# harveybc/gym-fx

Hardware: AMD Instinct MI355X
Metric: env-steps/sec (whole node) PPO EURUSD-1m 4096 vec-envs (higher is better)
Workload: dtype bf16; 1 GPU; model=PPO MLP(256,256) actor-critic bf16 MFMA, global_batch=524288, seq_len=32, parallelism=dp1, n_envs_per_gpu=4096, rollout_steps=128, obs_dim=260, preprocessor=feature_window_preprocessor, reward=pnl_reward, pairs=1

## Files before the change

### gymfx_amd/algo/ppo.py

```python
from __future__ import annotations

import time
from dataclasses import dataclass
from typing import Any, Dict, List

import torch

from ..envs.vec_env import VecFxEnv
from ..models.lstm import ActorCriticLSTM
from ..models.mlp import ActorCriticMLP
from ..ops import api


@dataclass
class PPOConfig:
    rollout_steps: int = 128
    ppo_epochs: int = 4
    minibatches: int = 8
    gamma: float = 0.99
    gae_lambda: float = 0.95
    clip_eps: float = 0.2
    ent_coef: float = 0.01
    vf_coef: float = 0.5
    lr: float = 3e-4
    max_grad_norm: float = 0.5
    seed: int = 0
    hidden: int = 256
    normalize_adv: bool = True
    shuffle_rows: bool = True
    use_graphs: bool = True
    policy: str = "mlp"
    bptt_len: int = 16
    fused_rollout: bool = False
    rollout_streams: int = 1
    fuse_sample: bool = True
    fuse_head: bool = False
    overlap_gather: bool = False
    fused_opt_tail: bool = True
    fused_head_bwd: bool = True

    @classmethod
    def from_config(cls, cfg: Dict[str, Any]) -> "PPOConfig":
        out = cls()
        mapping = {
            "rollout_steps": "rollout_steps",
            "ppo_epochs": "ppo_epochs",
            "minibatches": "minibatches",
            "gamma": "gamma",
            "gae_lambda": "gae_lambda",
            "clip_eps": "clip_eps",
            "ent_coef": "ent_coef",
            "vf_coef": "vf_coef",
            "lr": "learning_rate",
            "max_grad_norm": "max_grad_norm",
            "hidden": "hidden_size",
            "normalize_adv": "normalize_adv",
            "shuffle_rows": "shuffle_rows",
            "use_graphs": "use_graphs",
            "policy": "policy_model",
            "bptt_len": "bptt_len",
            "rollout_streams": "rollout_streams",
            "fused_rollout": "fused_rollout",
            "fuse_sample": "fuse_sample",
            "fuse_head": "fuse_head",
            "overlap_gather": "overlap_gather",
            "fused_opt_tail": "fused_opt_tail",
            "fused_head_bwd": "fused_head_bwd",
        }
        from ..config.merger import convert_type

        for attr, key in mapping.items():
            if cfg.get(key) is not None:
                cur = getattr(out, attr)
                val = convert_type(cfg[key]) if isinstance(cur, bool) else cfg[key]
                setattr(out, attr, type(cur)(val))
        if cfg.get("seed") is not None:
            out.seed = int(cfg["seed"])
        return out


class PPOTrainer:
    def __init__(self, env: VecFxEnv, cfg: PPOConfig, *, rank: int = 0,
                 world_size: int = 1, process_group=None):
        self.env = env
        self.cfg = cfg
        self.rank = rank
        self.world_size = world_size
        self.pg = process_group
        self.device = env.device
        if getattr(env.params, "action_space_mode", "discrete") != "discrete":
            raise ValueError(
                "PPO training uses the 3-way discrete head; set "
                "action_space_mode='discrete' (continuous mode is for "
                "external agents driving the env, reference "
                "env.py:343-360 coercion semantics)")

        N = env.n_envs
        T = cfg.rollout_steps
        D = env.obs_dim
        self.N, self.T, self.D = N, T, D
# ... 79 lines not shown
            self.logp_mb_s = [torch.empty(M, dtype=torch.float32, device=dev)
                              for _ in range(ns)]
            self.adv_mb_s = [torch.empty(M, dtype=torch.float32, device=dev)
                             for _ in range(ns)]
            self.ret_mb_s = [torch.empty(M, dtype=torch.float32, device=dev)
                             for _ in range(ns)]
            self.obs_mb = self.obs_mb_s[0]
            self.act_mb = self.act_mb_s[0]
            self.logp_mb = self.logp_mb_s[0]
            self.adv_mb = self.adv_mb_s[0]
            self.ret_mb = self.ret_mb_s[0]

        self.step_base = torch.zeros((), dtype=torch.int64, device=dev)
        self.mb_ctr = torch.zeros((), dtype=torch.int64, device=dev)
        self.sample_seed = cfg.seed * 1_000_003 + rank
        self.shuffle_seed = cfg.seed * 9973 + rank

        import os as _os
        self._fuse_gather = (
            not self.recurrent and self.device.type == "cuda"
            and cfg.shuffle_rows and not self._overlap
            and _os.environ.get("GYMFX_FUSE_GATHER", "0") == "1")
        self._fm = {"seed": self.shuffle_seed, "minibatches": cfg.minibatches,
                    "ctr_off": -1, "step_base": self.step_base,
                    "mb_ctr": self.mb_ctr}

        self._fused_tail = bool(cfg.fused_opt_tail) and (
            not self.recurrent
            or _os.environ.get("GYMFX_LSTM_OPT_TAIL", "0") == "1")
        self.model.fused_tail = self._fused_tail
        self.model.fuse_norm = (self._fused_tail and world_size <= 1
                                and cfg.max_grad_norm > 0)
        self._fused_head = bool(cfg.fused_head_bwd) and not self.recurrent
        self._loss_shards = (
            torch.zeros(64, 32, dtype=torch.float32, device=dev)
            if self._fused_head and self.device.type == "cuda" else None)
        self._mb_ticket = (
            torch.zeros((), dtype=torch.int32, device=dev)
            if self._fused_tail
            and _os.environ.get("GYMFX_GATHER_TICKET", "0") == "1" else None)

        self.global_step = 0
        self.update_count = 0
        self.use_graphs = bool(cfg.use_graphs) and self.device.type == "cuda"
        self._split = (self.device.type == "cuda" and cfg.rollout_streams > 1
                       and N % 2 == 0)
        self._fused = (self.device.type == "cuda" and cfg.fused_rollout
                       and not self.recurrent and cfg.hidden == 256)
        self._fuse_sample = (self.device.type == "cuda" and cfg.fuse_sample
                             and getattr(env, "_native", None) is not None
                             and env.params.action_space_mode != "continuous")
        self._fuse_head = (self._fuse_sample and cfg.fuse_head
                           and cfg.hidden % 8 == 0 and n_actions + 1 <= 8
                           and not cfg.fused_rollout)
        if self._split:
            self._s2 = torch.cuda.Stream()
            self.acts_half = [self.model.alloc_acts(N // 2),
                              self.model.alloc_acts(N // 2)]
        if self._overlap:
            self._gs = torch.cuda.Stream()
        self._graphs_ready = False
        self.g_rollout = None
        self.g_gather = None
        self.g_fwd_bwd = None
        self.g_opt = None
        from ..parallel.ddp import GradAllReducer
# ... 466 lines not shown
```

### gymfx_amd/config/defaults.py

```python
from __future__ import annotations

DEFAULT_VALUES = {
    "mode": "inference",
    "driver_mode": "buy_hold",
    "steps": 500,

    "data_feed_plugin": "default_data_feed",
    "broker_plugin": "default_broker",
    "strategy_plugin": "default_strategy",
    "preprocessor_plugin": "default_preprocessor",
    "reward_plugin": "pnl_reward",
    "metrics_plugin": "default_metrics",

    "input_data_file": "examples/data/eurusd.csv",
    "date_column": "DATE_TIME",
    "price_column": "CLOSE",
    "instrument": "EUR_USD",
    "timeframe": "M1",
    "headers": True,
    "max_rows": None,

    "window_size": 32,
    "initial_cash": 10000.0,
    "position_size": 1.0,
# ... 18 lines not shown
    "n_envs": 1,
    "device": "auto",
    "seed": None,
    "autoreset": False,
    "env_start_mode": "zero",
    "action_space_mode": "discrete",
    "continuous_action_threshold": 0.33,
    "min_equity": None,
    "financing_enabled": False,
    "rollover_rate_data": None,
    "financing_rate_data_file": None,
    "rollover_hour_utc": 22,
    "enforce_margin_preflight": False,

    "policy_model": "mlp",
    "hidden_size": 256,
    "rollout_steps": 128,
    "ppo_epochs": 4,
    "minibatches": 8,
    "bptt_len": 16,
    "learning_rate": 3e-4,
    "gamma": 0.99,
    "gae_lambda": 0.95,
    "clip_eps": 0.2,
    "ent_coef": 0.01,
    "vf_coef": 0.5,
    "max_grad_norm": 0.5,
    "train_updates": 10,
    "use_graphs": True,
    "fuse_sample": True,
    "overlap_gather": False,
    "fused_opt_tail": True,
    "fused_head_bwd": True,
    "checkpoint_file": None,
    "checkpoint_interval": 0,
    "resume": False,
    "trace_file": None,

    "serve_host": "127.0.0.1",
    "serve_port": 8400,

    "optimization_trials": 16,
    "optimization_steps": 256,
    "optimization_refine_trials": 0,
}
```

### gymfx_amd/models/mlp.py

```python
from __future__ import annotations

import math
from dataclasses import dataclass
from typing import Dict, Optional, Tuple

import torch

from ..ops import api


@dataclass
class _ParamSlice:
    name: str
    shape: Tuple[int, ...]
    sl: slice
    is_weight: bool


class ActorCriticMLP:
    def __init__(
        self,
        obs_dim: int,
        n_actions: int = 3,
        hidden: int = 256,
# ... 24 lines not shown
        self.n_params = off

        g = torch.Generator().manual_seed(seed)
        flat = torch.empty(off, dtype=torch.float32)
        for name, shape, is_w in dims:
            s = self.slices[name]
            if is_w:
                fan_in = shape[0]
                bound = 1.0 / math.sqrt(fan_in)
                flat[s.sl] = (torch.rand(s.sl.stop - s.sl.start, generator=g) * 2 - 1) * bound
            else:
                flat[s.sl] = 0.0
        self.params = flat.to(device)
        self.grads = torch.zeros_like(self.params)
        self.m = torch.zeros_like(self.params)
        self.v = torch.zeros_like(self.params)
        self.params_bf16 = self.params.to(torch.bfloat16)
        self._wt: Dict[str, torch.Tensor] = {}
        for name in ("W1", "W2", "W3"):
            s = self.slices[name]
            K_, N_ = s.shape
            self._wt[name] = torch.empty(N_, K_, dtype=torch.bfloat16, device=device)
        self._refresh_wt()
        self.adam_step = 0
        self.adam_ctr = torch.zeros((), dtype=torch.int32, device=device)
        self._clip_part = torch.zeros(256, dtype=torch.float32, device=device)
        self._clip_scale = torch.ones(1, dtype=torch.float32, device=device)
        self._wg_ws: Dict[str, Tuple[torch.Tensor, Optional[torch.Tensor]]] = {}
        self.wgrad_slabs = 64
        self.fused_tail = False
        self.fuse_norm = False
        self._adam_ticket = torch.zeros((), dtype=torch.int32, device=device)
        self._fin_segs = None

    def w(self, name: str) -> torch.Tensor:
        s = self.slices[name]
        return self.params_bf16[s.sl].view(*s.shape)

    def wt(self, name: str) -> torch.Tensor:
        return self._wt[name]

    def _refresh_wt(self) -> None:
        for name, t in self._wt.items():
            api.transpose_bf16(self.w(name), t)

    def f32(self, name: str) -> torch.Tensor:
        s = self.slices[name]
        return self.params[s.sl].view(*s.shape)

    def grad(self, name: str) -> torch.Tensor:
        s = self.slices[name]
        return self.grads[s.sl].view(*s.shape)

    def _wg_slabs(self, K: int, N: int) -> int:
        import os
        ov = os.environ.get("GYMFX_WGRAD_SLABS")
        if ov:
            return int(ov)
        tiles = ((K + 63) // 64) * ((N + 63) // 64)
        s = self.wgrad_slabs
        while tiles * s < 2048:
            s *= 2
        return s

    def _finalize_segments(self):
        if self._fin_segs is None:
# ... 5 lines not shown
                segs.append((db, N, S, self.slices[bn].sl.start, True))
            self._fin_segs = segs
        return self._fin_segs

    def _wg_workspace(self, name: str, K: int, N: int, want_db: bool):
        key = f"{name}:{K}x{N}"
        if key not in self._wg_ws:
            S = self._wg_slabs(K, N)
            dw = torch.empty(S, K, N, dtype=torch.float32, device=self.device)
            db = torch.empty(S, N, dtype=torch.float32, device=self.device) if want_db else None
            self._wg_ws[key] = (dw, db, S)
        return self._wg_ws[key]

    def alloc_acts(self, M: int) -> Dict[str, torch.Tensor]:
        dev = self.device
        return {
            "h1": torch.empty(M, self.hidden, dtype=torch.bfloat16, device=dev),
            "h2": torch.empty(M, self.hidden, dtype=torch.bfloat16, device=dev),
            "head": torch.empty(M, self.head_dim, dtype=torch.float32, device=dev),
        }

    def fused_step(self, obs_bf16: torch.Tensor, actions: torch.Tensor,
                   logp: torch.Tensor, value: torch.Tensor, *, seed: int,
                   step: int, step_base: torch.Tensor, row_offset: int = 0,
                   greedy: bool = False) -> None:
        from ..ops import native
        native.require().mlp_policy_rollout(
            obs_bf16, self.wt("W1"), self.f32("b1"), self.wt("W2"),
            self.f32("b2"), self.wt("W3"), self.f32("b3"), actions, logp,
            value, seed, step, step_base, row_offset, greedy)

    def forward(self, obs_bf16: torch.Tensor, acts: Dict[str, torch.Tensor],
                a_feistel: "Optional[dict]" = None) -> torch.Tensor:
        api.gemm(obs_bf16, self.wt("W1"), self.f32("b1"), acts["h1"], act=2,
                 trans_b=True, a_perm=a_feistel)
        api.gemm(acts["h1"], self.wt("W2"), self.f32("b2"), acts["h2"], act=2, trans_b=True)
        api.gemm(acts["h2"], self.wt("W3"), self.f32("b3"), acts["head"], act=0, trans_b=True)
        return acts["head"]

    def forward_hidden(self, obs_bf16: torch.Tensor,
                       acts: Dict[str, torch.Tensor]) -> torch.Tensor:
        api.gemm(obs_bf16, self.wt("W1"), self.f32("b1"), acts["h1"], act=2, trans_b=True)
        api.gemm(acts["h1"], self.wt("W2"), self.f32("b2"), acts["h2"], act=2, trans_b=True)
        return acts["h2"]

    def head_loss_backward(
        self,
        acts: Dict[str, torch.Tensor],
        actions: torch.Tensor,
        old_logp: torch.Tensor,
        adv: torch.Tensor,
        ret: torch.Tensor,
        dhead: torch.Tensor,
        scratch: Dict[str, torch.Tensor],
        *,
        clip_eps: float,
        ent_coef: float,
        vf_coef: float,
        inv_count: float,
        losses: Optional[torch.Tensor] = None,
    ) -> None:
        dw_p, db_p, slabs = self._wg_workspace("W3", self.hidden, self.head_dim, True)
        api.head_loss_bwd(
            acts["h2"], self.wt("W3"), self.w("W3"), self.f32("b3"), actions,
            old_logp, adv, ret, acts["head"], dhead, scratch["dh2"],
            self.grad("W3"), self.grad("b3"), workspace=(dw_p, db_p),
            slabs=slabs, reduce=not self.fused_tail, clip_eps=clip_eps,
            ent_coef=ent_coef, vf_coef=vf_coef, inv_count=inv_count,
            losses=losses)

    def backward(
        self,
        obs_bf16: torch.Tensor,
        acts: Dict[str, torch.Tensor],
        dhead: torch.Tensor,
        scratch: Dict[str, torch.Tensor],
        a_feistel: "Optional[dict]" = None,
        skip_head: bool = False,
    ) -> None:
        M = dhead.shape[0]
        dh2 = scratch["dh2"]
        dh1 = scratch["dh1"]
        red = not self.fused_tail
        if not skip_head:
            dw_p, db_p, slabs = self._wg_workspace("W3", self.hidden, self.head_dim, True)
            api.wgrad(acts["h2"], dhead, self.grad("W3"), self.grad("b3"),
                      workspace=(dw_p, db_p), slabs=slabs, reduce=red)
            api.gemm(dhead, self.w("W3"), None, dh2, Yact=acts["h2"], trans_b=True,
                     act=1, dact_tanh=True)
        dw_p, db_p, slabs = self._wg_workspace("W2", self.hidden, self.hidden, True)
        api.wgrad(acts["h1"], dh2, self.grad("W2"), self.grad("b2"),
                  workspace=(dw_p, db_p), slabs=slabs, reduce=red)
        api.gemm(dh2, self.w("W2"), None, dh1, Yact=acts["h1"], trans_b=True,
                 act=1, dact_tanh=True)
        dw_p, db_p, slabs = self._wg_workspace("W1", self.obs_dim, self.hidden, True)
        api.wgrad(obs_bf16, dh1, self.grad("W1"), self.grad("b1"),
                  workspace=(dw_p, db_p), slabs=slabs, x_perm=a_feistel,
                  reduce=red)
        if self.fused_tail:
            api.grads_finalize(self._finalize_segments(), self.grads,
                               self._clip_part if self.fuse_norm else None)

    def alloc_scratch(self, M: int) -> Dict[str, torch.Tensor]:
        dev = self.device
        return {
            "dh2": torch.empty(M, self.hidden, dtype=torch.bfloat16, device=dev),
            "dh1": torch.empty(M, self.hidden, dtype=torch.bfloat16, device=dev),
        }

    def adam(self, lr: float, *, beta1=0.9, beta2=0.999, eps=1e-8,
             max_grad_norm: float = 0.0) -> None:
        self.adam_step += 1
        clip = None
        if max_grad_norm and max_grad_norm > 0:
            clip = (self._clip_part, max_grad_norm)
        if self.fused_tail:
            api.adam_tail(self.params, self.grads, self.m, self.v,
                          self.params_bf16, lr=lr, beta1=beta1, beta2=beta2,
                          eps=eps, step_ctr=self.adam_ctr,
                          ticket=self._adam_ticket, clip=clip,
                          sumsq_done=self.fuse_norm,
                          mirrors=[(self.slices[n].sl.start, t)
                                   for n, t in self._wt.items()])
            return
        api.adam(self.params, self.grads, self.m, self.v, self.params_bf16,
                 lr=lr, beta1=beta1, beta2=beta2, eps=eps, step=self.adam_step,
                 step_ctr=self.adam_ctr, clip=clip)
# ... 26 lines not shown
```

### gymfx_amd/ops/api.py

```python
from __future__ import annotations

from typing import Optional, Sequence, Tuple

import os

import torch

from . import native

_LSTM_FUSED = os.environ.get("GYMFX_LSTM_FUSED", "1") != "0"
_LSTM_BWD_FUSED = os.environ.get("GYMFX_LSTM_BWD_FUSED", "0") == "1"


def _use_native(t: torch.Tensor) -> bool:
    if t.is_cuda:
        native.require()
        return True
    return False



def gemm(
    A: torch.Tensor,
    B: torch.Tensor,
    bias: Optional[torch.Tensor],
    C: torch.Tensor,
    *,
    Yact: Optional[torch.Tensor] = None,
    trans_b: bool = False,
    act: int = 1,
    dact_tanh: bool = False,
    accum: bool = False,
    a_perm: "Optional[dict]" = None,
) -> torch.Tensor:
    if _use_native(A):
        if a_perm is not None:
            native.require().gemm(A, B, bias, C, Yact, trans_b, act,
                                  dact_tanh, accum,
                                  ap_seed=a_perm["seed"],
                                  ap_minibatches=a_perm["minibatches"],
                                  ap_ctr_off=a_perm.get("ctr_off", 0),
                                  ap_step_base=a_perm["step_base"],
                                  ap_mb_ctr=a_perm["mb_ctr"])
            return C
        native.require().gemm(A, B, bias, C, Yact, trans_b, act, dact_tanh,
                              accum)
        return C
    if a_perm is not None:
        A = A[_perm_rows(A.shape[0], C.shape[0], a_perm)]
    a = A.to(torch.float32)
    b = B.to(torch.float32)
    if trans_b:
        b = b.t()
    out = a @ b
    if bias is not None:
        out = out + bias
    if act == 2:
        out = torch.tanh(out)
    if dact_tanh:
        y = Yact.to(torch.float32)
        out = out * (1.0 - y * y)
    if act == 0:
        if accum:
            C.add_(out)
        else:
            C.copy_(out)
    else:
        C.copy_(out.to(torch.bfloat16))
# ... 662 lines not shown
```

### gymfx_amd/ops/csrc/bindings.cpp

```cpp
#include <torch/extension.h>

#include <c10/hip/HIPStream.h>
#include <hip/hip_runtime.h>

#include <unordered_map>
#include <string>
#include <vector>

#include "env_common.h"
#include "mfma_dispatch.h"

namespace gymfx {

void launch_env_step(const EnvPtrs& P, const EnvParamsK& K, int env_lo,
                     int env_cnt, hipStream_t stream);
void launch_build_obs(const EnvPtrs& P, const EnvParamsK& K, int env_lo,
                      int env_cnt, hipStream_t stream);
void launch_env_step_obs(const EnvPtrs& P, const EnvParamsK& K, int env_lo,
                         int env_cnt, hipStream_t stream);
void launch_gemm(const void* A, const void* B, const float* bias, void* C,
                 const void* Yact, int M, int N, int K, bool trans_b, int act,
                 bool dact_tanh, bool add_bias, bool accum, hipStream_t stream,
                 const FeistelMap* fmp = nullptr);
void launch_lstm_cell_fwd(const void* gates_pre, const void* gates_h,
                          const float* c_prev, float* c_new, void* h_new,
                          const bool* done, void* h_masked, float* c_masked,
                          void* acts_out, int64_t M, int H,
                          hipStream_t stream);
void launch_lstm_cell_bwd(const void* acts, const float* c_prev,
                          const float* c_new, const void* dh_head,
                          const float* dh_next, const float* dc_next,
                          const bool* done, void* dgates, float* dc_prev,
                          int64_t M, int H, hipStream_t stream);
bool launch_lstm_gemm_cell_fwd(const void* A, const void* B,
                               const void* gates_pre, void* acts_out,
                               const float* c_prev, float* c_new, void* h_new,
                               const bool* done, void* h_masked,
                               float* c_masked, int M, int N, int K,
                               hipStream_t stream);
bool launch_lstm_bwd_fused(const void* acts, const float* c_prev,
                           const float* c_new, const void* dh_head,
                           const float* dh_next, const float* dc_next,
                           const bool* done, const void* B, void* dgates,
                           float* dc_prev, float* dh_prev, int M, int H,
                           hipStream_t stream);
void launch_mask_reset(void* h, float* c, const bool* done, int64_t M, int H,
                       hipStream_t stream);
void launch_masked_state(const void* h_raw, const float* c_raw,
                         const bool* done, void* h_in, float* c_in, int64_t M,
                         int H, hipStream_t stream);
void launch_mb_gather_seq(const void* obs_src, const int64_t* act_src,
                          const float* logp_src, const float* adv_src,
                          const float* ret_src, const bool* done_src,
                          const float* h0_src,
                          const float* c0_src, void* obs_mb, int64_t* act_mb,
                          float* logp_mb, float* adv_mb, float* ret_mb,
// ... 494 lines not shown
  const int N = trans_b ? (int)B.size(0) : (int)B.size(1);
  TORCH_CHECK((trans_b ? B.size(1) : B.size(0)) == K, "gemm K mismatch");
  TORCH_CHECK(C.size(1) == N && (C.size(0) == M || ap_step_base.has_value()),
              "gemm C shape");
  if (act == 0) check_f32(C, "C"); else check_bf16(C, "C");
  const float* bias_p = nullptr;
  if (bias.has_value()) {
    check_f32(*bias, "bias");
    TORCH_CHECK(bias->numel() == N, "bias numel");
    bias_p = bias->data_ptr<float>();
  }
  const void* y_p = nullptr;
  if (dact_tanh) {
    TORCH_CHECK(Yact.has_value(), "dact_tanh needs Yact");
    check_bf16(*Yact, "Yact");
    y_p = Yact->data_ptr();
  }
  if (ap_step_base.has_value()) {
    TORCH_CHECK(ap_mb_ctr.has_value(), "a_perm needs mb_ctr");
    const int M_mb = (int)C.size(0);
    gymfx::FeistelMap fm = make_fmap(A.size(0), M_mb, ap_seed,
                                     ap_minibatches, ap_ctr_off,
                                     *ap_step_base, *ap_mb_ctr);
    gymfx::launch_gemm(A.data_ptr(), B.data_ptr(), bias_p, C.data_ptr(), y_p,
                       M_mb, N, K, trans_b, (int)act, dact_tanh,
                       bias_p != nullptr, accum, cur_stream(), &fm);
    return;
  }
  gymfx::launch_gemm(A.data_ptr(), B.data_ptr(), bias_p, C.data_ptr(), y_p, M,
                     N, K, trans_b, (int)act, dact_tanh, bias_p != nullptr,
                     accum, cur_stream());
}

void lstm_cell_fwd_op(torch::Tensor gates_pre,
                      c10::optional<torch::Tensor> gates_h,
                      torch::Tensor c_prev,
                      torch::Tensor c_new, torch::Tensor h_new,
                      c10::optional<torch::Tensor> done,
                      c10::optional<torch::Tensor> h_masked,
                      c10::optional<torch::Tensor> c_masked,
                      c10::optional<torch::Tensor> acts_out) {
  check_bf16(gates_pre, "gates_pre");
  check_f32(c_prev, "c_prev");
  check_f32(c_new, "c_new");
  check_bf16(h_new, "h_new");
  const int64_t M = c_prev.size(0);
  const int H = (int)c_prev.size(1);
  TORCH_CHECK(gates_pre.size(0) == M && gates_pre.size(1) == 4 * H,
              "gates_pre shape");
  const void* gh = nullptr;
  if (gates_h.has_value()) {
    check_bf16(*gates_h, "gates_h");
    gh = gates_h->data_ptr();
  }
  const bool* done_p = nullptr;
  void* hm_p = nullptr;
  float* cm_p = nullptr;
  if (done.has_value()) {
    TORCH_CHECK(h_masked.has_value() && c_masked.has_value(),
                "done needs h_masked and c_masked outputs");
    TORCH_CHECK(done->scalar_type() == torch::kBool && done->numel() == M,
                "done must be bool [M]");
    check_bf16(*h_masked, "h_masked");
    check_f32(*c_masked, "c_masked");
    done_p = done->data_ptr<bool>();
    hm_p = h_masked->data_ptr();
// ... 616 lines not shown
  kn.bk64 = knob_or(bk64, pk.bk64);
  kn.n1 = knob_or(n1, pk.n1);
  const gymfx::GemmSel s =
      gymfx::select_gemm((int)M, (int)N, (int)K, trans_b, (int)act, dact_tanh,
                         add_bias, accum, a_perm, kn);
  TORCH_CHECK(gymfx::gemm_instantiated(s), "no gemm kernel instantiated for ",
              gymfx::gemm_name(s));
  return py::make_tuple(gymfx::gemm_name(s), py::make_tuple(s.gx, s.gy));
}

py::tuple wgrad_variant_op(int64_t M, int64_t N, int64_t K, int64_t slabs,
                           bool want_db, bool x_perm,
                           c10::optional<int64_t> big) {
  const gymfx::WgradSel s = gymfx::select_wgrad(
      (int)M, (int)N, (int)K, (int)slabs, want_db, x_perm,
      knob_or(big, gymfx::process_wgrad_big_knob()));
  return py::make_tuple(gymfx::wgrad_name(s),
                        py::make_tuple(s.gx, s.gy, s.gz));
}

}

PYBIND11_MODULE(TORCH_EXTENSION_NAME, m) {
  m.def("gemm", &gemm_op,
        "C = act(A @ B + bias); trans_b reads B as [N,K]; act 0=f32 1=bf16 "
        "2=tanh-bf16; dact_tanh multiplies by (1-Yact^2); accum does C += ",
        py::arg("A"), py::arg("B"), py::arg("bias"), py::arg("C"),
        py::arg("Yact") = py::none(), py::arg("trans_b") = false,
        py::arg("act") = 1, py::arg("dact_tanh") = false,
        py::arg("accum") = false, py::arg("ap_seed") = 0,
        py::arg("ap_minibatches") = 1, py::arg("ap_ctr_off") = 0,
        py::arg("ap_step_base") = py::none(),
        py::arg("ap_mb_ctr") = py::none());
  m.def("lstm_cell_fwd", &lstm_cell_fwd_op, py::arg("gates_pre"),
        py::arg("gates_h"), py::arg("c_prev"), py::arg("c_new"),
        py::arg("h_new"), py::arg("done") = py::none(),
        py::arg("h_masked") = py::none(), py::arg("c_masked") = py::none(),
        py::arg("acts_out") = py::none());
  m.def("lstm_gemm_cell_fwd", &lstm_gemm_cell_fwd_op,
        "fused h@Wh^T recurrent GEMM + LSTM cell epilogue; returns False "
        "when the shape has no fused kernel (caller falls back)",
        py::arg("A"), py::arg("B"), py::arg("gates_pre"),
        py::arg("acts_out"), py::arg("c_prev"), py::arg("c_new"),
        py::arg("h_new"), py::arg("done") = py::none(),
        py::arg("h_masked") = py::none(), py::arg("c_masked") = py::none());
  m.def("lstm_bwd_fused", &lstm_bwd_fused_op,
        "fused LSTM cell backward + dgates @ Wh recurrent dgrad; returns "
        "False when the shape has no fused kernel (caller falls back)",
        py::arg("acts"), py::arg("c_prev"),
        py::arg("c_new"), py::arg("dh_head"), py::arg("dh_next"),
        py::arg("dc_next"), py::arg("done"), py::arg("B"), py::arg("dgates"),
        py::arg("dc_prev"), py::arg("dh_prev") = py::none());
  m.def("lstm_cell_bwd", &lstm_cell_bwd_op, py::arg("acts"),
        py::arg("c_prev"), py::arg("c_new"), py::arg("dh_head"),
        py::arg("dh_next"), py::arg("dc_next"), py::arg("done"),
        py::arg("dgates"), py::arg("dc_prev"));
  m.def("mask_reset", &mask_reset_op, py::arg("h"), py::arg("c"),
        py::arg("done"));
  m.def("masked_state", &masked_state_op, py::arg("h_raw"), py::arg("c_raw"),
        py::arg("done"), py::arg("h_in"), py::arg("c_in"));
  m.def("mb_gather_seq", &mb_gather_seq_op, py::arg("obs_src"),
        py::arg("act_src"), py::arg("logp_src"), py::arg("adv_src"),
        py::arg("ret_src"), py::arg("done_src"), py::arg("h0_src"),
        py::arg("c0_src"),
        py::arg("obs_mb"), py::arg("act_mb"), py::arg("logp_mb"),
        py::arg("adv_mb"), py::arg("ret_mb"), py::arg("done_mb"),
// ... 96 lines not shown
```

### gymfx_amd/ops/csrc/mfma_dispatch.h

```cpp
#pragma once

#include <cstdint>
#include <cstdio>
#include <cstdlib>
#include <string>
#include <vector>

namespace gymfx {

struct GemmKnobs {
  int wide = -1;
  int bk64 = -1;
  int n1 = -1;
};

inline int knob_from_env(const char* name) {
  const char* e = getenv(name);
  return e ? atoi(e) : -1;
}

inline const GemmKnobs& process_gemm_knobs() {
  static const GemmKnobs k = [] {
    GemmKnobs v;
    v.wide = knob_from_env("GYMFX_GEMM_WIDE");
// ... 73 lines not shown
  X(true, 0, false, false, 8, true, 32, false)                                \
  X(false, 0, false, false, 2, true, 32, false)                               \
  X(false, 0, false, false, 4, true, 32, false)                               \
  X(false, 0, false, false, 8, true, 32, false)                               \
  X(true, 0, false, false, 1, false, 64, false)                               \
  X(true, 2, false, true, 2, false, 32, true)

inline bool gemm_sel_is(const GemmSel& s, bool tb, int act, bool dt, bool ab,
                        int nf, bool acc, int bk, bool perm) {
  return s.tb == tb && s.act == act && s.dt == dt && s.ab == ab &&
         s.nf == nf && s.acc == acc && s.bk == bk && s.perm == perm;
}

inline std::string gemm_name(bool tb, int act, bool dt, bool ab, int nf,
                             bool acc, int bk, bool perm) {
  char buf[96];
  snprintf(buf, sizeof buf, "tb%d_act%d_dt%d_ab%d_nf%d_bk%d_acc%d_perm%d",
           (int)tb, act, (int)dt, (int)ab, nf, bk, (int)acc, (int)perm);
  return buf;
}

inline std::string gemm_name(const GemmSel& s) {
  return gemm_name(s.tb, s.act, s.dt, s.ab, s.nf, s.acc, s.bk, s.perm);
}

inline bool gemm_instantiated(const GemmSel& s) {
#define GYMFX_X(TB, ACT, DT, AB, NF, ACC, BK, PERM)                           \
  if (gemm_sel_is(s, TB, ACT, DT, AB, NF, ACC, BK, PERM)) return true;
  GYMFX_GEMM_VARIANTS(GYMFX_X)
#undef GYMFX_X
  return false;
}

struct WgradSel {
  bool glds;
  bool db;
  int fk, fn;
  bool perm;
  int gx, gy, gz;
};

inline WgradSel select_wgrad(int M, int N, int K, int slabs, bool want_db,
                             bool x_perm, int big_knob) {
  const bool big =
      K >= 128 && N >= 128 &&
      (big_knob >= 0 ? big_knob != 0
                     : (int64_t)dispatch_ceil_div(K, 128) *
                               dispatch_ceil_div(N, 128) * slabs >=
                           384);
  const int m_per_slab = (M + slabs - 1) / slabs;
  const int TW = big ? 128 : 64;
  const bool glds_ok =
      N % TW == 0 && K >= TW && m_per_slab % 64 == 0 && M % slabs == 0;
  if (glds_ok) {
    if (big) {
      const int t44 = dispatch_ceil_div(K, 128);
      const int t54 = dispatch_ceil_div(K, 160);
      if (t54 < t44 && N <= 512)
        return {true, want_db, 5, 4, x_perm, t54, N / TW, slabs};
      return {true, want_db, 4, 4, x_perm, t44, N / TW, slabs};
    }
    return {true, want_db, 2, 2, x_perm, dispatch_ceil_div(K, 64), N / TW,
            slabs};
  }
  const int f = big ? 4 : 2;
  return {false, want_db, f, f, x_perm, dispatch_ceil_div(K, 32 * f),
// ... 52 lines not shown
```

### gymfx_amd/ops/csrc/ppo_kernels.hip

```cpp
#include "env_common.h"
#include "mfma_dispatch.h"

#include <hip/hip_bf16.h>

#include <algorithm>

namespace gymfx {

typedef __attribute__((ext_vector_type(8))) __bf16 bf16x8;
typedef __attribute__((ext_vector_type(4))) __bf16 bf16x4;
typedef __attribute__((ext_vector_type(4))) float f32x4;

GFX_DEV float bf2f(__bf16 v) { return (float)v; }
GFX_DEV __bf16 f2bf(float v) { return (__bf16)v; }

GFX_DEV float fast_tanh(float x) {
  x = fminf(fmaxf(x, -15.f), 15.f);
  const float e = __builtin_amdgcn_exp2f(x * 2.885390081777927f);
  return 1.f - 2.f * __builtin_amdgcn_rcpf(e + 1.f);
}

GFX_DEV uint32_t feistel_encrypt_once(uint32_t x, int half, uint32_t mask,
                                      uint64_t key) {
  uint32_t a = x & mask;
  uint32_t b = x >> half;
  for (int r = 0; r < 4; ++r) {
    const uint32_t f =
        (uint32_t)(splitmix64(key ^ ((uint64_t)r << 48) ^ (uint64_t)b)) & mask;
    const uint32_t t = b;
    b = a ^ f;
    a = t;
  }
  return (b << half) | a;
}

GFX_DEV uint32_t feistel_perm_idx(uint32_t i, uint32_t n, int half,
                                  uint64_t key) {
  const uint32_t mask = (1u << half) - 1u;
  uint32_t x = i;
  do {
    x = feistel_encrypt_once(x, half, mask, key);
  } while (x >= n);
  return x;
}

GFX_DEV uint64_t feistel_key(const FeistelMap& fm, uint32_t* mb) {
  const unsigned long long ctr =
      (unsigned long long)((long long)*fm.mb_ctr + fm.ctr_off);
  const uint32_t epoch = (uint32_t)(ctr / (unsigned)fm.minibatches);
  *mb = (uint32_t)(ctr % (unsigned)fm.minibatches);
  return splitmix64(fm.seed ^ (*fm.step_base * 0x9E3779B97F4A7C15ull) ^
                    ((uint64_t)epoch << 32));
// ... 165 lines not shown
      for (int mi = 0; mi < 2; ++mi)
        af[mi] = *reinterpret_cast<const bf16x8*>(
            &As[cur][wr * 32 + mi * 16 + row_a][ks * 32 + kseg * 8]);
      if (TRANS_B) {
        for (int ni = 0; ni < NFRAG; ++ni)
          bf[ni] = *reinterpret_cast<const bf16x8*>(
              &Bs[cur][wc * (16 * NFRAG) + ni * 16 + row_a][ks * 32 + kseg * 8]);
      } else {
        for (int ni = 0; ni < NFRAG; ++ni)
          for (int i = 0; i < 8; ++i)
            bf[ni][i] = Bs[cur][ks * 32 + kseg * 8 + i]
                          [wc * (16 * NFRAG) + ni * 16 + row_a];
      }
      for (int mi = 0; mi < 2; ++mi)
        for (int ni = 0; ni < NFRAG; ++ni)
          acc[mi][ni] = __builtin_amdgcn_mfma_f32_16x16x32_bf16(
              af[mi], bf[ni], acc[mi][ni], 0, 0, 0);
    }

    if (kt + 1 < ktiles && !nxt_glds) store_tile(1 - cur);
    __syncthreads();
  }

  const int crow_base = (lane >> 4) * 4;
  const int ccol = lane & 15;
  for (int mi = 0; mi < 2; ++mi) {
    for (int ni = 0; ni < NFRAG; ++ni) {
      const int gcol = bn + wc * (16 * NFRAG) + ni * 16 + ccol;
      if (gcol >= N) continue;
      for (int r = 0; r < 4; ++r) {
        const int grow = bm + wr * 32 + mi * 16 + crow_base + r;
        if (grow >= M) continue;
        float v = acc[mi][ni][r];
        if (ADD_BIAS) v += bias[gcol];
        if (ACT == 2) v = fast_tanh(v);
        if (DACT_TANH) {
          float y = bf2f(Yact[(int64_t)grow * N + gcol]);
          v *= (1.f - y * y);
        }
        if (ACT == 0) {
          float* cp = reinterpret_cast<float*>(C) + (int64_t)grow * N + gcol;
          *cp = ACCUM ? (*cp + v) : v;
        } else {
          reinterpret_cast<__bf16*>(C)[(int64_t)grow * N + gcol] = f2bf(v);
        }
      }
    }
  }
}

template <bool WANT_DB, int FK, int FN, bool A_PERM = false>
__global__ __launch_bounds__(256) void wgrad_glds_kernel(
    const __bf16* __restrict__ X, const __bf16* __restrict__ dY,
    float* __restrict__ dW_part, float* __restrict__ db_part,
    int M, int N, int K, int slabs, FeistelMap fm = FeistelMap{}) {
  constexpr int BKm = 64;
  constexpr int TK = 32 * FK, TN = 32 * FN;
  __shared__ __bf16 Xs[2][BKm][TK];
  __shared__ __bf16 Ys[2][BKm][TN];

  const int bk = blockIdx.x * TK;
  const int bn = blockIdx.y * TN;
  const int slab = blockIdx.z;
  const int tid = threadIdx.x;
  const int wave = tid >> 6, lane = tid & 63;
  const int wr = wave >> 1, wc = wave & 1;

  const int m_per_slab = (M + slabs - 1) / slabs;
  const int m_begin = slab * m_per_slab;
  const int m_end = min(M, m_begin + m_per_slab);
  const int nchunks = (m_end - m_begin) / BKm;
  f32x4 acc[FK][FN] = {};
  float db_acc = 0.f;

  uint64_t fkey = 0;
  uint32_t fmb = 0;
  if (A_PERM) fkey = feistel_key(fm, &fmb);
  auto x_row = [&](int gm) -> int64_t {
// ... 1863 lines not shown
                     0, stream, reinterpret_cast<const __bf16*>(obs_src),     \
                     act_src, logp_src, adv_src, ret_src,                     \
                     reinterpret_cast<__bf16*>(obs_mb), act_mb, logp_mb,      \
                     adv_mb, ret_mb, M, D, n, half, seed, minibatches,        \
                     step_base, mb_ctr, skip_obs, ticket)
  if (ticket) GATHER(true);
  else GATHER(false);
#undef GATHER
}

void launch_gemm(const void* A, const void* B, const float* bias, void* C,
                 const void* Yact, int M, int N, int K, bool trans_b, int act,
                 bool dact_tanh, bool add_bias, bool accum,
                 hipStream_t stream, const FeistelMap* fmp = nullptr) {
  const __bf16* a = reinterpret_cast<const __bf16*>(A);
  const __bf16* b = reinterpret_cast<const __bf16*>(B);
  const __bf16* y = reinterpret_cast<const __bf16*>(Yact);
  const GemmSel s = select_gemm(M, N, K, trans_b, act, dact_tanh, add_bias,
                                accum, fmp != nullptr, process_gemm_knobs());
  const dim3 grid(s.gx, s.gy), block(256);
  const FeistelMap fm = fmp ? *fmp : FeistelMap{};
#define GYMFX_X(TB, ACT, DT, AB, NF, ACC, BK, PERM)                           \
  if (gemm_sel_is(s, TB, ACT, DT, AB, NF, ACC, BK, PERM)) {                   \
    hipLaunchKernelGGL((gemm_kernel<TB, ACT, DT, AB, NF, ACC, BK, PERM>),     \
                       grid, block, 0, stream, a, b, bias, C, y, M, N, K,     \
                       fm);                                                   \
    return;                                                                   \
  }
  GYMFX_GEMM_VARIANTS(GYMFX_X)
#undef GYMFX_X
  abort();
}

void launch_slab_reduce(const float* dW_part, const float* db_part, float* dW,
                        float* db, int N, int K, int slabs, hipStream_t stream);

void launch_wgrad(const void* X, const void* dY, float* dW_part, float* db_part,
                  float* dW, float* db, int M, int N, int K, int slabs,
                  hipStream_t stream, const FeistelMap* fmp = nullptr,
                  bool reduce = true) {
  const __bf16* x = reinterpret_cast<const __bf16*>(X);
  const __bf16* dy = reinterpret_cast<const __bf16*>(dY);
  const WgradSel s = select_wgrad(M, N, K, slabs, db_part != nullptr,
                                  fmp != nullptr, process_wgrad_big_knob());
  const dim3 grid(s.gx, s.gy, s.gz);
  const FeistelMap fm = fmp ? *fmp : FeistelMap{};
  bool launched = false;
#define GYMFX_X(DB, FK, FN, PERM)                                             \
  if (wgrad_sel_is(s, true, DB, FK, FN, PERM)) {                              \
    hipLaunchKernelGGL((wgrad_glds_kernel<DB, FK, FN, PERM>), grid,           \
                       dim3(256), 0, stream, x, dy, dW_part, db_part, M, N,   \
                       K, slabs, fm);                                         \
    launched = true;                                                          \
  }
  GYMFX_WGRAD_GLDS_VARIANTS(GYMFX_X)
#undef GYMFX_X
#define GYMFX_X(DB, FK, FN, PERM)                                             \
  if (wgrad_sel_is(s, false, DB, FK, FN, PERM)) {                             \
    hipLaunchKernelGGL((wgrad_partial_kernel<DB, FK, FN, PERM>), grid,        \
                       dim3(256), 0, stream, x, dy, dW_part, db_part, M, N,   \
                       K, slabs, 0, fm);                                      \
    launched = true;                                                          \
  }
  GYMFX_WGRAD_PARTIAL_VARIANTS(GYMFX_X)
#undef GYMFX_X
  if (!launched) abort();
// ... 151 lines not shown
```

Before: 31.93 million env-steps/sec.

## Add weight-resident persistent GEMM kernel for tall N=256 MLP layers

Adds a persistent GEMM kernel for tall M×256 products with K≤264. Each workgroup loads the full 256×K weight matrix (and bias) into LDS once, then loops over 256-row groups of A, with the A fragments held in registers and the bias-tanh or dtanh epilogue fused in. It runs by default for batches of at least 65536 rows in the forward hidden layers and the W2 dgrad, and is skipped for permuted-A (Feistel-gathered) inputs. The goal is to stop re-streaming weight tiles from global memory for every output tile and to cut grid overhead. The cost is one large LDS allocation per block (about 135 KB) and low occupancy, at most one workgroup per CU.

Measured after the change: 34.04 million env-steps/sec (median of 6 runs). 6.6% higher.

```diff
diff --git a/gymfx_amd/algo/ppo.py b/gymfx_amd/algo/ppo.py
--- a/gymfx_amd/algo/ppo.py
+++ b/gymfx_amd/algo/ppo.py
@@ -38,6 +38,8 @@
     overlap_gather: bool = False
     fused_opt_tail: bool = True
     fused_head_bwd: bool = True
+    resident_gemm: bool = True
+    resident_min_rows: int = 65536
 
     @classmethod
     def from_config(cls, cfg: Dict[str, Any]) -> "PPOConfig":
@@ -66,6 +68,8 @@
             "overlap_gather": "overlap_gather",
             "fused_opt_tail": "fused_opt_tail",
             "fused_head_bwd": "fused_head_bwd",
+            "resident_gemm": "resident_gemm",
+            "resident_min_rows": "resident_min_rows",
         }
         from ..config.merger import convert_type
 
@@ -211,6 +215,9 @@
         self.model.fuse_norm = (self._fused_tail and world_size <= 1
                                 and cfg.max_grad_norm > 0)
         self._fused_head = bool(cfg.fused_head_bwd) and not self.recurrent
+        if not self.recurrent:
+            self.model.resident_gemm = bool(cfg.resident_gemm)
+            self.model.resident_min_rows = int(cfg.resident_min_rows)
         self._loss_shards = (
             torch.zeros(64, 32, dtype=torch.float32, device=dev)
             if self._fused_head and self.device.type == "cuda" else None)
diff --git a/gymfx_amd/config/defaults.py b/gymfx_amd/config/defaults.py
--- a/gymfx_amd/config/defaults.py
+++ b/gymfx_amd/config/defaults.py
@@ -74,6 +74,8 @@
     "overlap_gather": False,
     "fused_opt_tail": True,
     "fused_head_bwd": True,
+    "resident_gemm": True,
+    "resident_min_rows": 65536,
     "checkpoint_file": None,
     "checkpoint_interval": 0,
     "resume": False,
diff --git a/gymfx_amd/models/mlp.py b/gymfx_amd/models/mlp.py
--- a/gymfx_amd/models/mlp.py
+++ b/gymfx_amd/models/mlp.py
@@ -80,6 +80,11 @@
         self.fuse_norm = False
         self._adam_ticket = torch.zeros((), dtype=torch.int32, device=device)
         self._fin_segs = None
+        self.resident_gemm = False
+        self.resident_min_rows = 65536
+
+    def _resident(self, M: int) -> bool:
+        return self.resident_gemm and M >= self.resident_min_rows
 
     def w(self, name: str) -> torch.Tensor:
         s = self.slices[name]
@@ -151,16 +156,21 @@
 
     def forward(self, obs_bf16: torch.Tensor, acts: Dict[str, torch.Tensor],
                 a_feistel: "Optional[dict]" = None) -> torch.Tensor:
+        res = self._resident(acts["h1"].shape[0])
         api.gemm(obs_bf16, self.wt("W1"), self.f32("b1"), acts["h1"], act=2,
-                 trans_b=True, a_perm=a_feistel)
-        api.gemm(acts["h1"], self.wt("W2"), self.f32("b2"), acts["h2"], act=2, trans_b=True)
+                 trans_b=True, a_perm=a_feistel, resident=res)
+        api.gemm(acts["h1"], self.wt("W2"), self.f32("b2"), acts["h2"], act=2,
+                 trans_b=True, resident=res)
         api.gemm(acts["h2"], self.wt("W3"), self.f32("b3"), acts["head"], act=0, trans_b=True)
         return acts["head"]
 
     def forward_hidden(self, obs_bf16: torch.Tensor,
                        acts: Dict[str, torch.Tensor]) -> torch.Tensor:
-        api.gemm(obs_bf16, self.wt("W1"), self.f32("b1"), acts["h1"], act=2, trans_b=True)
-        api.gemm(acts["h1"], self.wt("W2"), self.f32("b2"), acts["h2"], act=2, trans_b=True)
+        res = self._resident(acts["h1"].shape[0])
+        api.gemm(obs_bf16, self.wt("W1"), self.f32("b1"), acts["h1"], act=2,
+                 trans_b=True, resident=res)
+        api.gemm(acts["h1"], self.wt("W2"), self.f32("b2"), acts["h2"], act=2,
+                 trans_b=True, resident=res)
         return acts["h2"]
 
     def head_loss_backward(
@@ -211,7 +221,7 @@
         api.wgrad(acts["h1"], dh2, self.grad("W2"), self.grad("b2"),
                   workspace=(dw_p, db_p), slabs=slabs, reduce=red)
         api.gemm(dh2, self.w("W2"), None, dh1, Yact=acts["h1"], trans_b=True,
-                 act=1, dact_tanh=True)
+                 act=1, dact_tanh=True, resident=self._resident(dh2.shape[0]))
         dw_p, db_p, slabs = self._wg_workspace("W1", self.obs_dim, self.hidden, True)
         api.wgrad(obs_bf16, dh1, self.grad("W1"), self.grad("b1"),
                   workspace=(dw_p, db_p), slabs=slabs, x_perm=a_feistel,
diff --git a/gymfx_amd/ops/api.py b/gymfx_amd/ops/api.py
--- a/gymfx_amd/ops/api.py
+++ b/gymfx_amd/ops/api.py
@@ -32,8 +32,16 @@
     dact_tanh: bool = False,
     accum: bool = False,
     a_perm: "Optional[dict]" = None,
+    resident: bool = False,
 ) -> torch.Tensor:
     if _use_native(A):
+        if resident and a_perm is None:
+            ext = native.require()
+            N = B.shape[0] if trans_b else B.shape[1]
+            if ext.gemm_resident_ok(A.shape[0], N, A.shape[1], trans_b, act,
+                                    dact_tanh, bias is not None, accum):
+                ext.gemm_resident(A, B, bias, C, Yact, act, dact_tanh)
+                return C
         if a_perm is not None:
             native.require().gemm(A, B, bias, C, Yact, trans_b, act,
                                   dact_tanh, accum,
diff --git a/gymfx_amd/ops/csrc/bindings.cpp b/gymfx_amd/ops/csrc/bindings.cpp
--- a/gymfx_amd/ops/csrc/bindings.cpp
+++ b/gymfx_amd/ops/csrc/bindings.cpp
@@ -22,6 +22,9 @@
                  const void* Yact, int M, int N, int K, bool trans_b, int act,
                  bool dact_tanh, bool add_bias, bool accum, hipStream_t stream,
                  const FeistelMap* fmp = nullptr);
+void launch_gemm_resident(const void* A, const void* Wt, const float* bias,
+                          void* C, const void* Yact, int M, int K, int act,
+                          bool dact_tanh, int max_blocks, hipStream_t stream);
 void launch_lstm_cell_fwd(const void* gates_pre, const void* gates_h,
                           const float* c_prev, float* c_new, void* h_new,
                           const bool* done, void* h_masked, float* c_masked,
@@ -582,6 +585,49 @@
                      accum, cur_stream());
 }
 
+void gemm_resident_op(torch::Tensor A, torch::Tensor Wt,
+                      c10::optional<torch::Tensor> bias, torch::Tensor C,
+                      c10::optional<torch::Tensor> Yact, int64_t act,
+                      bool dact_tanh, int64_t max_blocks) {
+  check_bf16(A, "A");
+  check_bf16(Wt, "Wt");
+  check_bf16(C, "C");
+  TORCH_CHECK(A.dim() == 2 && Wt.dim() == 2 && C.dim() == 2,
+              "gemm_resident operands must be 2-d");
+  const int64_t M = A.size(0), K = A.size(1), N = Wt.size(0);
+  TORCH_CHECK(Wt.size(1) == K, "gemm_resident K mismatch");
+  TORCH_CHECK(C.size(0) == M && C.size(1) == N, "gemm_resident C shape");
+  TORCH_CHECK(gymfx::gemm_resident_ok(M, N, K, true, (int)act, dact_tanh,
+                                      bias.has_value(), false),
+              "gemm_resident: shape/epilogue not supported (M=", M, " N=", N,
+              " K=", K, " act=", act, " dact_tanh=", dact_tanh, ")");
+  TORCH_CHECK(max_blocks >= 0, "max_blocks must be >= 0");
+  auto aligned = [](const torch::Tensor& t, uintptr_t a) {
+    return reinterpret_cast<uintptr_t>(t.data_ptr()) % a == 0;
+  };
+  TORCH_CHECK(aligned(A, 8) && aligned(Wt, 8) && aligned(C, 8),
+              "gemm_resident operands must be 8-byte aligned");
+  const float* bias_p = nullptr;
+  if (bias.has_value()) {
+    check_f32(*bias, "bias");
+    TORCH_CHECK(bias->numel() == N, "bias numel");
+    TORCH_CHECK(aligned(*bias, 16), "gemm_resident bias must be 16-byte aligned");
+    bias_p = bias->data_ptr<float>();
+  }
+  const void* y_p = nullptr;
+  if (dact_tanh) {
+    TORCH_CHECK(Yact.has_value(), "dact_tanh needs Yact");
+    check_bf16(*Yact, "Yact");
+    TORCH_CHECK(Yact->dim() == 2 && Yact->size(0) == M && Yact->size(1) == N,
+                "gemm_resident Yact shape");
+    TORCH_CHECK(aligned(*Yact, 8), "gemm_resident Yact must be 8-byte aligned");
+    y_p = Yact->data_ptr();
+  }
+  gymfx::launch_gemm_resident(A.data_ptr(), Wt.data_ptr(), bias_p,
+                              C.data_ptr(), y_p, (int)M, (int)K, (int)act,
+                              dact_tanh, (int)max_blocks, cur_stream());
+}
+
 void lstm_cell_fwd_op(torch::Tensor gates_pre,
                       c10::optional<torch::Tensor> gates_h,
                       torch::Tensor c_prev,
@@ -1264,6 +1310,19 @@
         py::arg("ap_minibatches") = 1, py::arg("ap_ctr_off") = 0,
         py::arg("ap_step_base") = py::none(),
         py::arg("ap_mb_ctr") = py::none());
+  m.def("gemm_resident", &gemm_resident_op,
+        "weight-resident tall GEMM, N=256, K<=264: C = tanh(A @ Wt^T + bias) "
+        "(act=2) or (A @ Wt^T) * (1-Yact^2) (act=1, dact_tanh); bitwise the "
+        "gemm() result; max_blocks caps the grid (0 = one workgroup per CU)",
+        py::arg("A"), py::arg("Wt"), py::arg("bias"), py::arg("C"),
+        py::arg("Yact") = py::none(), py::arg("act") = 2,
+        py::arg("dact_tanh") = false, py::arg("max_blocks") = 0);
+  m.def("gemm_resident_ok", &gymfx::gemm_resident_ok,
+        "host predicate: can gemm_resident run this shape and epilogue",
+        py::arg("M"), py::arg("N"), py::arg("K"), py::arg("trans_b") = true,
+        py::arg("act") = 2, py::arg("dact_tanh") = false,
+        py::arg("add_bias") = true, py::arg("accum") = false,
+        py::arg("a_perm") = false);
   m.def("lstm_cell_fwd", &lstm_cell_fwd_op, py::arg("gates_pre"),
         py::arg("gates_h"), py::arg("c_prev"), py::arg("c_new"),
         py::arg("h_new"), py::arg("done") = py::none(),
diff --git a/gymfx_amd/ops/csrc/mfma_dispatch.h b/gymfx_amd/ops/csrc/mfma_dispatch.h
--- a/gymfx_amd/ops/csrc/mfma_dispatch.h
+++ b/gymfx_amd/ops/csrc/mfma_dispatch.h
@@ -129,6 +129,28 @@
   return false;
 }
 
+constexpr int RESIDENT_N = 256;
+constexpr int RESIDENT_LD = 264;
+constexpr int RESIDENT_GROUP = 256;
+
+inline bool gemm_resident_ok(int64_t M, int64_t N, int64_t K, bool trans_b,
+                             int act, bool dact_tanh, bool add_bias,
+                             bool accum, bool a_perm = false) {
+  if (M < 1 || M > INT32_MAX - RESIDENT_GROUP) return false;
+  if (N != RESIDENT_N || K < 4 || K > RESIDENT_LD || K % 4 != 0) return false;
+  if (!trans_b || accum || a_perm) return false;
+  const bool fwd = act == 2 && add_bias && !dact_tanh;
+  const bool dgrad = act == 1 && dact_tanh && !add_bias;
+  return fwd || dgrad;
+}
+
+inline int gemm_resident_grid(int64_t M, int n_cus, int max_blocks) {
+  const int64_t groups = (M + RESIDENT_GROUP - 1) / RESIDENT_GROUP;
+  int64_t cap = max_blocks > 0 ? max_blocks : n_cus;
+  if (cap < 1) cap = 1;
+  return (int)(groups < cap ? groups : cap);
+}
+
 struct WgradSel {
   bool glds;
   bool db;
diff --git a/gymfx_amd/ops/csrc/ppo_kernels.hip b/gymfx_amd/ops/csrc/ppo_kernels.hip
--- a/gymfx_amd/ops/csrc/ppo_kernels.hip
+++ b/gymfx_amd/ops/csrc/ppo_kernels.hip
@@ -18,6 +18,12 @@
   x = fminf(fmaxf(x, -15.f), 15.f);
   const float e = __builtin_amdgcn_exp2f(x * 2.885390081777927f);
   return 1.f - 2.f * __builtin_amdgcn_rcpf(e + 1.f);
+}
+
+GFX_DEV float epi_bias_tanh(float v, float b) { return fast_tanh(v + b); }
+GFX_DEV float epi_dtanh(float v, __bf16 yact) {
+  const float y = bf2f(yact);
+  return v * (1.f - y * y);
 }
 
 GFX_DEV uint32_t feistel_encrypt_once(uint32_t x, int half, uint32_t mask,
@@ -249,18 +255,183 @@
         const int grow = bm + wr * 32 + mi * 16 + crow_base + r;
         if (grow >= M) continue;
         float v = acc[mi][ni][r];
-        if (ADD_BIAS) v += bias[gcol];
-        if (ACT == 2) v = fast_tanh(v);
-        if (DACT_TANH) {
-          float y = bf2f(Yact[(int64_t)grow * N + gcol]);
-          v *= (1.f - y * y);
+        if (ADD_BIAS && ACT == 2) {
+          v = epi_bias_tanh(v, bias[gcol]);
+        } else {
+          if (ADD_BIAS) v += bias[gcol];
+          if (ACT == 2) v = fast_tanh(v);
         }
+        if (DACT_TANH) v = epi_dtanh(v, Yact[(int64_t)grow * N + gcol]);
         if (ACT == 0) {
           float* cp = reinterpret_cast<float*>(C) + (int64_t)grow * N + gcol;
           *cp = ACCUM ? (*cp + v) : v;
         } else {
           reinterpret_cast<__bf16*>(C)[(int64_t)grow * N + gcol] = f2bf(v);
         }
+      }
+    }
+  }
+}
+
+template <int EPI, int NFULL_CT, bool TAIL_CT = false>
+__global__ __launch_bounds__(512) void gemm_resident_kernel(
+    const __bf16* __restrict__ A, const __bf16* __restrict__ Wt,
+    const float* __restrict__ bias, __bf16* __restrict__ C,
+    const __bf16* __restrict__ Yact, int M, int K) {
+  constexpr int N = RESIDENT_N, LD = RESIDENT_LD, GROUP = RESIDENT_GROUP;
+  __shared__ __align__(16) __bf16 Ws[N * LD + 2 * N];
+  float* bias_s = reinterpret_cast<float*>(&Ws[N * LD]);
+
+  const int tid = threadIdx.x;
+  const int wave = tid >> 6;
+  const int lane = tid & 63;
+  const int row_l = lane & 15;
+  const int kseg = lane >> 4;
+
+  const int nfull = NFULL_CT >= 0 ? NFULL_CT : K / 32;
+  const int ktail = NFULL_CT >= 0 ? (int)TAIL_CT : K - nfull * 32;
+  const int kpad8 = (K + 7) & ~7;
+
+  const int kt = nfull * 32 + kseg * 8;
+  const bool t_lo = kt + 4 <= K, t_hi = kt + 8 <= K;
+  const int t_lo_off = t_lo ? kt : 0, t_hi_off = t_hi ? kt + 4 : 0;
+  const bool w_tv = kt < kpad8;
+  const int w_t_off = w_tv ? kt : 0;
+
+  const __bf16* pa[2];
+  auto set_rows = [&](int g) {
+    for (int mi = 0; mi < 2; ++mi) {
+      const int r = min(g * GROUP + wave * 32 + mi * 16 + row_l, M - 1);
+      pa[mi] = A + (int64_t)r * K;
+    }
+  };
+  auto load_full = [&](int mi, int kc) {
+    return *reinterpret_cast<const bf16x8*>(pa[mi] + kc * 32 + kseg * 8);
+  };
+  auto load_tail = [&](int mi) {
+    bf16x4 lo = *reinterpret_cast<const bf16x4*>(pa[mi] + t_lo_off);
+    bf16x4 hi = *reinterpret_cast<const bf16x4*>(pa[mi] + t_hi_off);
+    if (!t_lo) lo = bf16x4{};
+    if (!t_hi) hi = bf16x4{};
+    return __builtin_shufflevector(lo, hi, 0, 1, 2, 3, 4, 5, 6, 7);
+  };
+
+  constexpr int LATE = (NFULL_CT >= 4 && TAIL_CT) ? 2 : 0;
+  constexpr int NA = NFULL_CT >= 0 ? (NFULL_CT > 0 ? NFULL_CT : 1) : 1;
+  bf16x8 a[NA][2];
+  bf16x8 atail[2];
+  auto load_group = [&](int g) {
+    set_rows(g);
+    if (NFULL_CT >= 0) {
+      for (int kc = 0; kc < NFULL_CT - LATE; ++kc)
+        for (int mi = 0; mi < 2; ++mi) a[kc][mi] = load_full(mi, kc);
+    } else if (nfull > 0) {
+      for (int mi = 0; mi < 2; ++mi) a[0][mi] = load_full(mi, 0);
+    }
+    if (NFULL_CT < 0)
+      for (int mi = 0; mi < 2; ++mi) atail[mi] = load_tail(mi);
+  };
+
+  load_group(blockIdx.x);
+
+  {
+    constexpr int FILL_IT = (N * (LD / 8) + 511) / 512;
+    const int gpr = NFULL_CT >= 0 ? NFULL_CT * 4 + (TAIL_CT ? 1 : 0) : kpad8 / 8;
+    const int total = N * gpr;
+    bf16x4 flo[FILL_IT], fhi[FILL_IT];
+    for (int j = 0; j < FILL_IT; ++j) {
+      const int e = min(tid + j * 512, total - 1);
+      const int n = e / gpr;
+      const int k = (e - n * gpr) * 8;
+      const __bf16* src = Wt + (int64_t)n * K + k;
+      const bool hv = k + 8 <= K;
+      flo[j] = *reinterpret_cast<const bf16x4*>(src);
+      fhi[j] = *reinterpret_cast<const bf16x4*>(src + (hv ? 4 : 0));
+    }
+    for (int j = 0; j < FILL_IT; ++j) {
+      const int e = tid + j * 512;
+      const int n = e / gpr;
+      const int k = (e - n * gpr) * 8;
+      if (e < total) {
+        const bf16x4 hi = k + 8 <= K ? fhi[j] : bf16x4{};
+        *reinterpret_cast<bf16x8*>(&Ws[n * LD + k]) =
+            __builtin_shufflevector(flo[j], hi, 0, 1, 2, 3, 4, 5, 6, 7);
+      }
+    }
+    if (EPI == 0 && tid < N) bias_s[tid] = bias[tid];
+  }
+  __syncthreads();
+
+  const __bf16* wrow = &Ws[row_l * LD + kseg * 8];
+  f32x4 acc[2][16];
+  auto mma_chunk = [&](int k0, const bf16x8& a0, const bf16x8& a1) {
+    for (int ni = 0; ni < 16; ++ni) {
+      if (ni % 4 == 0) __builtin_amdgcn_sched_barrier(0);
+      const bf16x8 wf =
+          *reinterpret_cast<const bf16x8*>(wrow + ni * 16 * LD + k0);
+      acc[0][ni] = __builtin_amdgcn_mfma_f32_16x16x32_bf16(wf, a0, acc[0][ni],
+                                                           0, 0, 0);
+      acc[1][ni] = __builtin_amdgcn_mfma_f32_16x16x32_bf16(wf, a1, acc[1][ni],
+                                                           0, 0, 0);
+    }
+  };
+
+  for (int g = blockIdx.x; g * GROUP < M; g += gridDim.x) {
+    if (g != (int)blockIdx.x) load_group(g);
+    for (int mi = 0; mi < 2; ++mi)
+      for (int ni = 0; ni < 16; ++ni) acc[mi][ni] = f32x4{};
+
+    if (NFULL_CT >= 0) {
+      for (int kc = 0; kc < NFULL_CT; ++kc) {
+        const int slot = kc >= NFULL_CT - LATE ? kc - (NFULL_CT - LATE) : kc;
+        mma_chunk(kc * 32, a[slot][0], a[slot][1]);
+        if (kc < LATE)
+          for (int mi = 0; mi < 2; ++mi)
+            a[kc][mi] = load_full(mi, NFULL_CT - LATE + kc);
+        if (TAIL_CT && kc == LATE)
+          for (int mi = 0; mi < 2; ++mi) atail[mi] = load_tail(mi);
+      }
+    } else {
+      for (int kc = 0; kc < nfull; ++kc) {
+        const int kn = min(kc + 1, nfull - 1);
+        const bf16x8 n0 = load_full(0, kn), n1 = load_full(1, kn);
+        mma_chunk(kc * 32, a[0][0], a[0][1]);
+        a[0][0] = n0;
+        a[0][1] = n1;
+      }
+    }
+    if (ktail) {
+      for (int ni = 0; ni < 16; ++ni) {
+        bf16x8 wf = *reinterpret_cast<const bf16x8*>(
+            &Ws[(ni * 16 + row_l) * LD + w_t_off]);
+        if (!w_tv) wf = bf16x8{};
+        acc[0][ni] = __builtin_amdgcn_mfma_f32_16x16x32_bf16(
+            wf, atail[0], acc[0][ni], 0, 0, 0);
+        acc[1][ni] = __builtin_amdgcn_mfma_f32_16x16x32_bf16(
+            wf, atail[1], acc[1][ni], 0, 0, 0);
+      }
+    }
+
+    for (int mi = 0; mi < 2; ++mi) {
+      const int grow = g * GROUP + wave * 32 + mi * 16 + row_l;
+      if (grow >= M) continue;
+      const int64_t o = (int64_t)grow * N + kseg * 4;
+      bf16x4 y[16];
+      if (EPI == 1)
+        for (int ni = 0; ni < 16; ++ni)
+          y[ni] = *reinterpret_cast<const bf16x4*>(&Yact[o + ni * 16]);
+      for (int ni = 0; ni < 16; ++ni) {
+        bf16x4 out;
+        if (EPI == 0) {
+          const f32x4 b =
+              *reinterpret_cast<const f32x4*>(&bias_s[ni * 16 + kseg * 4]);
+          for (int r = 0; r < 4; ++r)
+            out[r] = f2bf(epi_bias_tanh(acc[mi][ni][r], b[r]));
+        } else {
+          for (int r = 0; r < 4; ++r)
+            out[r] = f2bf(epi_dtanh(acc[mi][ni][r], y[ni][r]));
+        }
+        *reinterpret_cast<bf16x4*>(&C[o + ni * 16]) = out;
       }
     }
   }
@@ -2190,6 +2361,40 @@
   abort();
 }
 
+void launch_gemm_resident(const void* A, const void* Wt, const float* bias,
+                          void* C, const void* Yact, int M, int K, int act,
+                          bool dact_tanh, int max_blocks, hipStream_t stream) {
+  if (!gemm_resident_ok(M, RESIDENT_N, K, true, act, dact_tanh,
+                        bias != nullptr, false))
+    abort();
+  static const int n_cus = [] {
+    int dev = 0, n = 0;
+    if (hipGetDevice(&dev) != hipSuccess ||
+        hipDeviceGetAttribute(&n, hipDeviceAttributeMultiprocessorCount,
+                              dev) != hipSuccess)
+      return 256;
+    return n;
+  }();
+  const dim3 grid(gemm_resident_grid(M, n_cus, max_blocks)), block(512);
+  const __bf16* a = reinterpret_cast<const __bf16*>(A);
+  const __bf16* w = reinterpret_cast<const __bf16*>(Wt);
+  const __bf16* y = reinterpret_cast<const __bf16*>(Yact);
+  __bf16* c = reinterpret_cast<__bf16*>(C);
+#define RESIDENT(EPI, NF, TAIL)                                               \
+  hipLaunchKernelGGL((gemm_resident_kernel<EPI, NF, TAIL>), grid, block, 0,   \
+                     stream, a, w, bias, c, y, M, K)
+#define RESIDENT_EPI(EPI)                                                     \
+  do {                                                                        \
+    if (K == 256) RESIDENT(EPI, 8, false);                                    \
+    else if (K > 256) RESIDENT(EPI, 8, true);                                 \
+    else RESIDENT(EPI, -1, false);                                            \
+  } while (0)
+  if (dact_tanh) RESIDENT_EPI(1);
+  else RESIDENT_EPI(0);
+#undef RESIDENT_EPI
+#undef RESIDENT
+}
+
 void launch_slab_reduce(const float* dW_part, const float* db_part, float* dW,
                         float* db, int N, int K, int slabs, hipStream_t stream);
 
```
